# slinderman/theano_pyglm

Measured on AMD Instinct MI355X. Metric: population ll+grad evals/sec (N neurons x T bins), higher is better.
Workload: dtype f64

## Files before the change

theano_pyglm_amd/csrc/pglm_capi.hip:

```cpp
#include "pglm_kernels.hip.h"
#include "../../include/pyglm_hip.h"

#include <algorithm>
#include <cmath>
#include <cstdio>
#include <cstring>
#include <map>
#include <mutex>
#include <string>
#include <thread>
#include <type_traits>
#include <vector>

static thread_local std::string g_err;
static int fail(int code, const std::string& msg)
{
    g_err = msg;
    return code;
}
static thread_local std::vector<std::string>* g_dry = nullptr;
static thread_local std::vector<std::string>* g_rec = nullptr;
#define HIPCHK(expr)                                                                         \
    do {                                                                                     \
        hipError_t e_ = (expr);                                                              \
// ... 677 lines not shown
    sp.P = P; sp.Bt = h->sepBt; sp.Rt = h->sepRt; sp.npost = npost; sp.xs = xs;
    sp.Tstim = h->sepT; sp.nT = h->nT; sp.t_lo = t_lo; sp.t_hi = t_hi; sp.dt = h->dt; sp.dt_stim = h->sep_dt_stim;
    sp.X = X;
    const int nblk = (int)((t_hi - t_lo + PGL_SEP_TB - 1) / PGL_SEP_TB);
    hipLaunchKernelGGL(k_sep_conv_fwd, dim3(nblk, npost), dim3(256), (size_t)(2 * h->sepRt + PGL_SEP_TB) * 8,
                       h->stream, sp);
    HIPCHK(hipGetLastError());
    return PGL_OK;
}

static int sep_backward(pgl_handle h, const SepParams& sp, double* d_grad)
{
    if (g_dry) return PGL_OK;
    const int npost = sp.npost, Rt = h->sepRt;
    const int nblk = (int)((sp.t_hi - sp.t_lo + PGL_SEP_TB - 1) / PGL_SEP_TB);
    ENSURE(h->spart, (size_t)nblk * npost * Rt * 8);
    hipLaunchKernelGGL(k_sep_corr, dim3(nblk, npost), dim3(256), (size_t)(Rt + 2 * PGL_SEP_TB) * 8, h->stream, sp,
                       (double*)h->spart.p);
    HIPCHK(hipGetLastError());
    hipLaunchKernelGGL(k_sep_wt_grad, dim3(npost), dim3(64), 0, h->stream, sp, (const double*)h->spart.p, nblk,
                       d_grad);
    HIPCHK(hipGetLastError());
    const long long s_lo = std::max<long long>(0, sp.t_lo - Rt), nS = sp.t_hi - s_lo;
    ENSURE(h->Qb, (size_t)npost * nS * 8);
    ENSURE(h->Qf, (size_t)npost * h->sepT * 8);
    const int nblk_s = (int)((nS + PGL_SEP_TB - 1) / PGL_SEP_TB);
    hipLaunchKernelGGL(k_sep_conv_bwd, dim3(nblk_s, npost), dim3(256), (size_t)(2 * Rt + PGL_SEP_TB) * 8, h->stream,
                       sp, (double*)h->Qb.p, s_lo, nS);
    HIPCHK(hipGetLastError());
    hipLaunchKernelGGL(k_sep_interp_T, dim3((unsigned)((h->sepT + 255) / 256), npost), dim3(256), 0, h->stream, sp,
                       (const double*)h->Qb.p, s_lo, nS, (double*)h->Qf.p);
    HIPCHK(hipGetLastError());
    return launch_gemm_nt(h, (const double*)h->Qf.p, (int)h->sepT, (const double*)h->zfT.p, (int)h->sepT,
                          d_grad + 1 + h->sepBt, sp.P, npost, h->sepBx, (int)h->sepT);
}

static int launch_gemm_mfma(pgl_handle h, const double* A, long long sam, long long sak, const double* B,
                            long long sbn, long long sbk, double* C, long long scm, long long scn, int M, int N, int K)
{
    const int mb = (M + 15) / 16;
    if ((long long)mb * ((N + 63) / 64) >= 128)
        return launch_gemm_mfma_nt<4>(h, A, sam, sak, 0, B, sbn, sbk, 0, C, scm, scn, 0, M, N, K, 1);
    return launch_gemm_mfma_nt<1>(h, A, sam, sak, 0, B, sbn, sbk, 0, C, scm, scn, 0, M, N, K, 1);
}

static int launch_sepf_any(pgl_handle h, int which, const SepfParams& sp)
{
    if (h->sepJ == 5 && h->sepBTp == 3) launch_sepf<5, 3>(which, sp, h->stream);
    else launch_sepf<8, 4>(which, sp, h->stream);
    HIPCHK(hipGetLastError());
    return PGL_OK;
}

static int sepf_forward(pgl_handle h, const Plan& pl, const double* d_theta, SepfParams& sp, bool fused_fwd)
{
    if (g_dry) return PGL_OK;
    const int P = 1 + h->Dstim + h->Kimp, ldy = pl.nPT * 16;
    ENSURE(h->YfT, (size_t)h->sepT * ldy * 8);
    int rc = PGL_OK;
    const double* wx = d_theta + 1 + h->sepBt;
    if (gemm_aligned(h->zf.p, h->sepBx) && gemm_aligned(wx, P)) {
        rc = launch_gemm_kc<4, 1, 8>(h, (const double*)h->zf.p, (long long)h->sepBx, wx, (long long)P, (double*)h->YfT.p,
                                     (long long)ldy, 1LL, (int)h->sepT, pl.npost, h->sepBx);
    } else {
        rc = launch_gemm_mfma(h, wx, P, 1, (const double*)h->zfT.p, 1, h->sepT, (double*)h->YfT.p, 1, ldy, pl.npost,
                              (int)h->sepT, h->sepBx);
    }
    if (rc) return rc;
    sp.Ctab = (const double*)h->sepC.p; sp.YfT = (const double*)h->YfT.p; sp.theta = d_theta;
    sp.X = (double*)h->Xbuf.p; sp.Hb = nullptr; sp.wpart = nullptr; sp.QvT = nullptr; sp.grad = nullptr;
    sp.D = nullptr; sp.B0 = sp.B1 = 0; sp.SL = 0; sp.tilesPerChunk = 0;
    sp.P = P; sp.Bt = h->sepBt; sp.M = h->sepM; sp.q = h->sepq; sp.npost = pl.npost; sp.nPT = pl.nPT; sp.ldy = ldy;
    sp.tile0 = pl.tile0; sp.nTiles = pl.nTiles; sp.Tstim = h->sepT;
    const long long tb = (long long)pl.tile0 * 16, te = tb + (long long)pl.nTiles * 16;
    sp.F0 = tb / h->sepq; sp.F1 = (te - 1) / h->sepq;
    if (fused_fwd) return PGL_OK;
    return launch_sepf_any(h, 0, sp);
}

static int sepf_backward(pgl_handle h, SepfParams& sp, double* d_grad, bool fused_bwd = false, int* nwt = nullptr)
{
    if (g_dry) return PGL_OK;
    const long long nF = sp.F1 - sp.F0 + 1;
    ENSURE(h->QvT, (size_t)h->sepT * sp.ldy * 8);
    int rc = PGL_OK;
    if (fused_bwd) {
        const int nblk = (int)((h->sepT + 15) / 16);
        ENSURE(h->wpart, (size_t)nblk * 3 * sp.ldy * 8);
        sp.wpart = (double*)h->wpart.p; sp.QvT = (double*)h->QvT.p; sp.grad = d_grad;
        hipLaunchKernelGGL(k_sepf_finish_d, dim3((unsigned)nblk), dim3(1024), 0, h->stream, sp);
        HIPCHK(hipGetLastError());
        if (nwt) *nwt = nblk;
    } else {
        ENSURE(h->Hb, (size_t)nF * h->sepJ * sp.ldy * 8);
        ENSURE(h->wpart, (size_t)nF * h->sepBTp * sp.ldy * 8);
        sp.Hb = (double*)h->Hb.p; sp.wpart = (double*)h->wpart.p; sp.QvT = (double*)h->QvT.p; sp.grad = d_grad;
        rc = launch_sepf_any(h, 1, sp);
        if (!rc) rc = launch_sepf_any(h, 2, sp);
    }
    if (rc) return rc;
    if (gemm_aligned(h->zfT.p, h->sepT)) {
        return launch_gemm_kc<1, 0, 16>(h, (const double*)h->zfT.p, (long long)h->sepT, (const double*)h->QvT.p,
                                        (long long)sp.ldy, d_grad + 1 + h->sepBt, 1LL, (long long)sp.P, h->sepBx, sp.npost,
                                        (int)h->sepT);
    }
    return launch_gemm_mfma(h, (const double*)h->zf.p, 1, h->sepBx, (const double*)h->QvT.p, 1, sp.ldy,
                            d_grad + 1 + h->sepBt, 1, sp.P, h->sepBx, sp.npost, (int)h->sepT);
}

int pgl_sta(pgl_handle h, const double* stim, int64_t Tstim, int D, double dt_stim, int L,
            const int* neurons, int n_sel, double* A_out)
{
    if (!h || !stim) return fail(PGL_ERR_ARG, "null argument");
    if (!h->have_spikes) return fail(PGL_ERR_STATE, "pgl_set_spikes_* has not been called");
    if (Tstim <= 0 || D <= 0 || L <= 0 || !(dt_stim > 0)) return fail(PGL_ERR_ARG, "bad stimulus description");
    const int nSel = neurons ? n_sel : h->N;
    if (nSel <= 0 || nSel > 65535) return fail(PGL_ERR_ARG, "bad neuron selection");
    std::vector<int> eoff((size_t)2 * nSel);
    for (int i = 0; i < nSel; ++i) {
        const int n = neurons ? neurons[i] : i;
        if (n < 0 || n >= h->N) return fail(PGL_ERR_ARG, "neuron index out of range");
        eoff[2 * i] = h->h_ptr[n];
        eoff[2 * i + 1] = h->h_ptr[n + 1];
    }
    const long long LD = (long long)L * D;
    const long long xb = (LD + 255) / 256;
    if (xb > 0x7fffffffLL) return fail(PGL_ERR_UNSUPPORTED, "L*D too large");
    int echunks = (int)std::min<long long>(64, std::max<long long>(1, 4096 / (xb * nSel)));
    HIPCHK(hipSetDevice(h->device));
    DevBuf dstim, distim, deoff, dpart, dA;
    auto cleanup = [&]() { release(dstim); release(distim); release(deoff); release(dpart); release(dA); };
    auto keep = [&]() {
        release(h->staA);
        h->staA = dA;
        dA = DevBuf();
        h->sta_n = nSel; h->sta_L = L; h->sta_D = D;
    };
    const double ratio = dt_stim / h->dt;
    const long long q = llround(ratio);
    const bool frame_rate = q >= 1 && std::fabs(ratio - (double)q) <= 1e-9 * ratio && (Tstim % 2) == 0 && Tstim >= 2 &&
                            (long long)nSel * L * Tstim <= (1ll << 28) && h->opt_sepf != 7;
    int rc = ensure(dstim, (size_t)Tstim * D * 8);
    if (!rc && !frame_rate) rc = ensure(distim, (size_t)h->nT * D * 8);
    if (!rc) rc = ensure(deoff, eoff.size() * sizeof(int));
    if (!rc && !frame_rate) rc = ensure(dpart, (size_t)echunks * nSel * LD * 8);
    if (!rc) rc = ensure(dA, (size_t)nSel * LD * 8);
    if (rc) { cleanup(); return rc; }
    hipError_t e = hipMemcpyAsync(dstim.p, stim, (size_t)Tstim * D * 8, hipMemcpyHostToDevice, h->stream);
    if (e == hipSuccess)
        e = hipMemcpyAsync(deoff.p, eoff.data(), eoff.size() * sizeof(int), hipMemcpyHostToDevice, h->stream);
    if (frame_rate && e == hipSuccess) {
        DevBuf dW, dscale;
        std::vector<double> scale((size_t)nSel);
        for (int i = 0; i < nSel; ++i) {
            double cnt = 0.0;
            for (int j = eoff[2 * i]; j < eoff[2 * i + 1]; ++j) cnt += (double)h->h_ev[j].y;
            scale[i] = (h->dt / dt_stim) / cnt;
        }
        rc = ensure(dW, (size_t)nSel * L * Tstim * 8);
        if (!rc) rc = ensure(dscale, (size_t)nSel * 8);
// ... 280 lines not shown
                           (const uint8_t*)h->S.p, h->N, n_lo, p0.npost, (long long)h->t_lo, (long long)h->t_hi, rows, h->nlin,
                           h->dt, (double*)h->tmpA.p, (double*)h->tmpB.p, h->cur_pidx);
    HIPCHK(hipGetLastError());
    if (rr.row1 > h->t_hi) {
        hipLaunchKernelGGL(k_rows_zero, dim3(64), dim3(256), 0, h->stream, (double*)h->Xbuf.p, rr.xs, (long long)h->t_hi, rr.row1);
        HIPCHK(hipGetLastError());
    }
    hipLaunchKernelGGL(k_rows_reduce, dim3(p0.npost), dim3(64), 0, h->stream, (const double*)h->tmpA.p,
                       (const double*)h->tmpB.p, nblk, p0.npost, 1 + h->Dstim + h->Kimp, d_ll, d_out);
    HIPCHK(hipGetLastError());
    return PGL_OK;
}

static int backward_slices(pgl_handle h, const std::vector<Slice>& slices, const std::vector<Plan>& plans, int n_lo,
                           const double* d_theta, const double* d_Weff, double* d_ll, double* d_out)
{
    for (size_t i = 0; i < slices.size(); ++i) {
        int rc = launch_prep(h, plans[i], slices[i], n_lo, d_theta, d_Weff);
        if (rc) return rc;
        FusedParams fp;
        fill_params(h, plans[i], slices[i], n_lo, true, 2, fp);
        hipError_t e = launch_plan(plans[i], fp, h->stream);
        if (e != hipSuccess) return fail(PGL_ERR_HIP, std::string("backward launch: ") + hipGetErrorString(e));
        rc = launch_finalize_grad(h, plans[i], slices[i], n_lo, d_Weff, d_ll, d_out);
        if (rc) return rc;
    }
    return PGL_OK;
}

static int enqueue_ll_grad(pgl_handle h, int n_lo, int n_hi, const double* d_theta,
                           const double* d_Weff, double* d_ll, double* d_grad)
{
    KernelRecord record(h);
    std::vector<Slice> slices;
    std::vector<Plan> plans;
    bool sepf = false, sliced = false, wide = false;
    {
        int rc = select_plans(h, n_lo, n_hi, slices, plans, sepf, sliced, &wide);
        if (rc) return rc;
    }
    {
        int rc = ensure_partials(h, plans, d_grad != nullptr);
        if (rc) return rc;
    }

    const bool rec = h->opt_timing > 0 && (h->call_no++ % h->opt_timing) == 0;
    if (rec) {
        h->ev = h->evr[h->ev_launches % pgl_context::NEV];
        HIPCHK(hipEventRecord(h->ev[0], h->stream));
    }
    if (sepf) {
        const Plan& pl = plans[0];
        const bool direct = plan_reads_theta(pl);
        int rc = direct ? PGL_OK : launch_prep(h, pl, slices[0], n_lo, d_theta, d_Weff);
        if (rc) return rc;
        ENSURE(h->Xbuf, (size_t)pl.nTiles * pl.nPT * 256 * 8);
        rc = ensure_plan_images(h, pl);
        if (rc) return rc;
        if (rec) HIPCHK(hipEventRecord(h->ev[1], h->stream));
        SepfParams sp{};
        const bool fused_fwd = pl.version == 7 && fused7_built(pl.KT, pl.nw7, 2) && h->sepA_ok && h->opt_sepf != 3;
        const bool fused_bwd = fused_fwd && d_grad && fused7_built(pl.KT, pl.nw7, 3) && h->opt_sepf != 4;
        rc = sepf_forward(h, pl, d_theta, sp, fused_fwd);
        if (rc) return rc;
        if (fused_bwd && !g_dry) {
            const long long q = h->sepq, M = h->sepM;
            const long long tE = (long long)pl.tile0 + pl.nTiles - 1;
            sp.B0 = std::max<long long>(((long long)pl.tile0 * 16) / q - M, 0);
            sp.B1 = std::max<long long>((tE * 16) / q - M, 0);
            const long long span = ((M + 1) * q + 15) / 16 + 1;
            sp.SL = (int)(span / pl.tilesPerChunk) + 2;
            sp.tilesPerChunk = pl.tilesPerChunk;
            ENSURE(h->sepD, (size_t)(sp.B1 - sp.B0 + 1) * sp.SL * pl.nPT * 320 * 8);
            sp.D = (const double*)h->sepD.p;
        }
        FusedParams fp;
        fill_params(h, pl, slices[0], n_lo, d_grad != nullptr, 0, fp);
        if (direct) {
            fp.theta = d_theta;
            fp.Weff = d_Weff;
        }
        if (fused_fwd) {
            fp.sepA = (const double*)h->sepA.p; fp.sepZ = sp.YfT; fp.sepTheta = d_theta; fp.sepT = h->sepT;
            fp.sepLdy = sp.ldy; fp.sepQ = h->sepq; fp.sepM = h->sepM; fp.sepNH = h->sepNH; fp.sepG = h->sepGs;
            fp.sepBt = h->sepBt;
        }
        if (fused_bwd) {
            fp.sepAT = (const double*)h->sepAT.p; fp.sepD = (double*)h->sepD.p; fp.sepB0 = sp.B0; fp.sepSL = sp.SL;
        }
        hipError_t e = hipSuccess;
        if (pl.version == 5) {
            e = launch_fused5(pl, fp, h->stream, 1, 1);
            if (e == hipSuccess && d_grad) e = launch_fused5(pl, fp, h->stream, 2);
        } else {
            e = launch_fused7(pl, fp, h->stream, fused_bwd ? 3 : (fused_fwd ? 2 : 1));
        }
        if (e != hipSuccess) return fail(PGL_ERR_HIP, std::string("fused launch: ") + hipGetErrorString(e));
        if (d_grad) {
            int nwt = 0;
            rc = sepf_backward(h, sp, d_grad, fused_bwd, &nwt);
            if (rc) return rc;
            if (rec) HIPCHK(hipEventRecord(h->ev[2], h->stream));
            rc = launch_finalize_grad(h, pl, slices[0], n_lo, d_Weff, d_ll, d_grad, true, 0, -1, nullptr,
                                      fused_bwd ? (const double*)h->wpart.p : nullptr, nwt, sp.ldy);
            if (rc) return rc;
        } else {
            if (rec) HIPCHK(hipEventRecord(h->ev[2], h->stream));
            rc = launch_finalize_ll(h, pl, d_ll, d_grad);
            if (rc) return rc;
        }
    } else if (!sliced) {
        const Plan& pl = plans[0];
        const bool direct = plan_reads_theta(pl);
        int rc = direct ? PGL_OK : launch_prep(h, pl, slices[0], n_lo, d_theta, d_Weff);
        if (rc) return rc;
        if ((pl.version == 4 || pl.version == 5) && d_grad) {
            rc = ensure_tile_slab(h, pl);
            if (rc) return rc;
        }
        rc = ensure_plan_images(h, pl);
        if (rc) return rc;
        FusedParams fp;
        fill_params(h, pl, slices[0], n_lo, d_grad != nullptr, 0, fp);
        if (direct) {
            fp.theta = d_theta;
            fp.Weff = d_Weff;
        }
        if (rec) HIPCHK(hipEventRecord(h->ev[1], h->stream));
        hipError_t e = launch_plan(pl, fp, h->stream);
        if (e != hipSuccess) return fail(PGL_ERR_HIP, std::string("fused launch: ") + hipGetErrorString(e));
        if (rec) HIPCHK(hipEventRecord(h->ev[2], h->stream));
        rc = d_grad ? launch_finalize_grad(h, pl, slices[0], n_lo, d_Weff, d_ll, d_grad, true) : launch_finalize_ll(h, pl, d_ll, d_grad);
        if (rc) return rc;
    } else if (wide) {
        const Plan& p0 = plans[0];
        const size_t S = slices.size();
        ENSURE(h->Xbuf, (size_t)p0.nTiles * p0.nPT * 256 * 8);
        std::vector<int> slot(S);
        for (size_t i = 0; i < S; ++i) {
            int rc = ensure_feature_images(h, plans[i].ktl, plans[i].kth, p0.tile0, p0.nTiles, &slices[i], (int)i);
            if (rc) return rc;
            slot[i] = h->img_cur;
        }
        if (rec) HIPCHK(hipEventRecord(h->ev[1], h->stream));
        auto params = [&](const size_t i, FusedParams& fp) {
            h->img_cur = slot[i];
            fill_params(h, plans[i], slices[i], n_lo, d_grad != nullptr, 0, fp);
        };
        for (size_t i = 0; i < S; ++i) {
            int rc = launch_prep(h, plans[i], slices[i], n_lo, d_theta, d_Weff);
            if (rc) return rc;
// ... 1566 lines not shown
```

theano_pyglm_amd/csrc/pglm_reduce.hip.h:

```cpp
#pragma once
__global__ void k_prep_w(const double* __restrict__ theta, const double* __restrict__ Weff,
                         double* __restrict__ Wfrag, double* __restrict__ bias, int N, int B,
                         int Dstim, int Kimp, int Ktot, int KS, int n_lo, int npost, int nPT,
                         int pair, int Nall, int np0, int DsAll, int ds0, const int* __restrict__ pidx)
{
    const int P = 1 + DsAll + Nall * B;
    const long long total = (long long)nPT * KS * 64;
    for (long long i = blockIdx.x * (long long)blockDim.x + threadIdx.x; i < total;
         i += (long long)gridDim.x * blockDim.x) {
        const int lane = (int)(i & 63);
        const int ks = (int)((i >> 6) % KS);
        const int pt = (int)((i >> 6) / KS);
        const int k = 4 * ks + (lane >> 4);
        const int n = 16 * pt + (lane & 15);
        double v = 0.0;
        if (n < npost && k < Ktot) {
            if (k < Kimp) {
                const int npre = np0 + k / B;
                v = theta[(size_t)n * P + 1 + DsAll + np0 * B + k] * Weff[(size_t)npre * Nall + (pidx ? pidx[n] : n_lo + n)];
            } else {
                v = theta[(size_t)n * P + 1 + ds0 + (k - Kimp)];
            }
        }
        const long long o = pair ? (((long long)pt * (KS / 2) + (ks >> 1)) * 64 + lane) * 2 + (ks & 1) : i;
        Wfrag[o] = v;
    }
    for (int n = blockIdx.x * blockDim.x + threadIdx.x; n < nPT * 16; n += gridDim.x * blockDim.x)
        bias[n] = (n < npost) ? theta[(size_t)n * P] : 0.0;
}

__device__ __forceinline__ void pgl_reduce_ll(const double* __restrict__ llpart, const double* __restrict__ gbpart,
                                              double* __restrict__ ll_out, double* __restrict__ grad_out,
                                              const int n, const int P, const int nPT, const int nChunks,
                                              const int nsub, double (*red)[64])
{
    const int nthr = 256, t = (int)threadIdx.x, lane = t & 63, w = t >> 6, nw = 4;
    const int total = nChunks * nsub;
    const double* __restrict__ lp = llpart + (size_t)n * total;
    const double* __restrict__ gp = gbpart + (size_t)n * total;
    double sl[4] = {0.0, 0.0, 0.0, 0.0}, sg[4] = {0.0, 0.0, 0.0, 0.0};
    for (int i0 = t; i0 < total && t < nthr; i0 += 4 * nthr) {
#pragma unroll
        for (int j = 0; j < 4; ++j) {
            const int i = i0 + j * nthr;
            if (i < total) {
                sl[j] += lp[i];
                sg[j] += gp[i];
            }
        }
    }
    double a = (sl[0] + sl[1]) + (sl[2] + sl[3]), b = (sg[0] + sg[1]) + (sg[2] + sg[3]);
    for (int o = 32; o > 0; o >>= 1) {
        a += __shfl_xor(a, o, 64);
        b += __shfl_xor(b, o, 64);
    }
    if (lane == 0 && w < nw) {
        red[w][0] = a;
        red[w][1] = b;
    }
    __syncthreads();
    if (t == 0) {
        double x = 0.0, y = 0.0;
        for (int j = 0; j < nw; ++j) {
            x += red[j][0];
            y += red[j][1];
        }
        ll_out[n] = x;
        if (grad_out != nullptr) grad_out[(size_t)n * P] = y;
    }
}

__global__ __launch_bounds__(1024) void k_finalize(const double* __restrict__ Gpart, const double* __restrict__ llpart,
                           const double* __restrict__ gbpart, const double* __restrict__ Weff,
                           double* __restrict__ ll_out, double* __restrict__ grad_out, int N, int B,
                           int Dstim, int Kimp, int Ktot, int KT, int n_lo, int npost, int nPT,
                           int nChunks, int Nall, int np0, int DsAll, int ds0, int nsub, int kt0,
                           int nkt, const int* __restrict__ pidx, const double* __restrict__ wtpart = nullptr,
                           int nwt = 0, int ldy = 0, int Bt = 0)
{
    const int P = 1 + DsAll + Nall * B;
    const int nwf = (int)(blockDim.x >> 6);
    const long long nfrag = (long long)nPT * nkt * 256;
    const int gblocks = (int)((nfrag + 63) / 64);
    __shared__ double red[16][64];
    if ((int)blockIdx.x >= gblocks) {
        if (nsub <= 0) return;
        const int n = (int)blockIdx.x - gblocks;
        if (n >= npost) {
            const int bt = n - npost;
            if (wtpart == nullptr || bt >= Bt || grad_out == nullptr) return;
            const int lane = (int)(threadIdx.x & 63), w = (int)(threadIdx.x >> 6);
            double a[4] = {0.0, 0.0, 0.0, 0.0};
            if (lane < ldy) {
                int i = w, u = 0;
                for (; i < nwt; i += nwf, ++u) a[u & 3] += wtpart[((size_t)i * 3 + bt) * ldy + lane];
            }
            red[w][lane] = (a[0] + a[1]) + (a[2] + a[3]);
            __syncthreads();
            if (w == 0 && lane < npost) {
                double v = 0.0;
                for (int j = 0; j < nwf; ++j) v += red[j][lane];
                grad_out[(size_t)lane * P + 1 + bt] = v;
            }
            return;
        }
        pgl_reduce_ll(llpart, gbpart, ll_out, grad_out, n, P, nPT, nChunks, nsub, red);
        return;
    }
    if (grad_out == nullptr) return;
    const int lane = (int)(threadIdx.x & 63), w = (int)(threadIdx.x >> 6);
    const long long gid = blockIdx.x * 64LL + lane;
    const int r = (int)((gid >> 6) & 3);
    const int kt = kt0 + (int)((gid >> 8) % nkt);
    const int pt = (int)((gid >> 8) / nkt);
    const int k = 16 * kt + (lane >> 4) + 4 * r;
    const int n = 16 * pt + (lane & 15);
    const bool live = gid < nfrag && n < npost && k < Ktot;
    double s = 0.0;
    if (live) {
        const int per = (nChunks + nwf - 1) / nwf;
        const int c0 = w * per, c1 = (c0 + per < nChunks) ? c0 + per : nChunks;
        const double* gp = Gpart + (((size_t)pt * KT + kt) * 4 + r) * ((size_t)nChunks * 64) + lane;
        double a[8] = {0.0, 0.0, 0.0, 0.0, 0.0, 0.0, 0.0, 0.0};
        int c = c0;
        for (; c + 8 <= c1; c += 8) {
#pragma unroll
            for (int j = 0; j < 8; ++j) a[j] += gp[(size_t)(c + j) * 64];
        }
        for (int j = 0; c < c1; ++c, ++j) a[j] += gp[(size_t)c * 64];
        s = ((a[0] + a[1]) + (a[2] + a[3])) + ((a[4] + a[5]) + (a[6] + a[7]));
    }
    red[w][lane] = s;
    __syncthreads();
    if (w == 0 && live) {
        s = 0.0;
        for (int j = 0; j < nwf; ++j) s += red[j][lane];
        if (k < Kimp) {
            const int npre = np0 + k / B;
            grad_out[(size_t)n * P + 1 + DsAll + np0 * B + k] = s * Weff[(size_t)npre * Nall + (pidx ? pidx[n] : n_lo + n)];
        } else {
            grad_out[(size_t)n * P + 1 + ds0 + (k - Kimp)] = s;
        }
    }
}

__global__ __launch_bounds__(256) void k_finalize_ll(const double* __restrict__ llpart,
                                                     const double* __restrict__ gbpart,
                                                     double* __restrict__ ll_out,
                                                     double* __restrict__ grad_out, int P, int npost,
                                                     int nPT, int nChunks, int nsub)
{
    __shared__ double red[16][64];
    const int n = blockIdx.x;
    if (n >= npost) return;
    pgl_reduce_ll(llpart, gbpart, ll_out, grad_out, n, P, nPT, nChunks, nsub, red);
}

__global__ __launch_bounds__(256) void k_rows_epilogue(double* __restrict__ Xbuf, int xstride,
                                                       const double* __restrict__ bias,
                                                       const uint8_t* __restrict__ S, int Nall,
                                                       int n_lo, int npost, long long t_lo,
                                                       long long t_hi, int rows, int nlin, double dt,
                                                       double* __restrict__ llp,
                                                       double* __restrict__ gbp,
                                                       const int* __restrict__ pidx)
{
    const int n = blockIdx.y * 256 + threadIdx.x;
    if (n >= npost) return;
    const long long t0 = t_lo + (long long)blockIdx.x * rows;
    long long t1 = t0 + rows;
    if (t1 > t_hi) t1 = t_hi;
    const double b = bias[n];
    double ll = 0.0, gb = 0.0;
    for (long long t = t0; t < t1; ++t) {
        const double x = Xbuf[t * xstride + n] + b;
        const double s = (double)S[t * Nall + (pidx ? pidx[n] : n_lo + n)];
        double term, res;
        pgl_rate_terms(x, s, nlin, dt, term, res, PGL_C);
        ll += term;
        gb += res;
        Xbuf[t * xstride + n] = res;
    }
    llp[(size_t)blockIdx.x * npost + n] = ll;
    gbp[(size_t)blockIdx.x * npost + n] = gb;
}

__global__ void k_rows_zero(double* __restrict__ Xbuf, int xstride, long long r0, long long r1)
{
    const long long total = (r1 - r0) * xstride;
    for (long long i = blockIdx.x * (long long)blockDim.x + threadIdx.x; i < total;
         i += (long long)gridDim.x * blockDim.x)
        Xbuf[r0 * xstride + i] = 0.0;
}

__global__ __launch_bounds__(64) void k_rows_reduce(const double* __restrict__ llp,
                                                    const double* __restrict__ gbp, int nblk,
// ... 19 lines not shown
```

theano_pyglm_amd/csrc/pglm_stim.hip.h:

```cpp
#pragma once
__global__ void k_stim_project(const double* __restrict__ stim, long long Tstim, int D,
                               double dt_stim, double dt, const double* __restrict__ basis_x,
                               int Bx, double* __restrict__ zx, long long nT)
{
    const long long total = nT * Bx;
    for (long long i = blockIdx.x * (long long)blockDim.x + threadIdx.x; i < total;
         i += (long long)gridDim.x * blockDim.x) {
        const long long t = i / Bx;
        const int bx = (int)(i - t * Bx);
        const double x = dt * (double)t;
        long long i0 = (long long)floor(x / dt_stim);
        if (i0 > Tstim - 2) i0 = Tstim - 2;
        if (i0 < 0) i0 = 0;
        while (i0 + 1 < Tstim - 1 && dt_stim * (double)(i0 + 1) <= x) ++i0;
        while (i0 > 0 && dt_stim * (double)i0 > x) --i0;
        const double x0 = dt_stim * (double)i0, x1 = dt_stim * (double)(i0 + 1);
        const bool beyond = (Tstim < 2) || (x >= dt_stim * (double)(Tstim - 1));
        double acc = 0.0;
        const int d_lo = (basis_x == nullptr) ? bx : 0;
        const int d_hi = (basis_x == nullptr) ? bx + 1 : D;
        for (int d = d_lo; d < d_hi; ++d) {
            double v;
            if (beyond) {
                v = stim[(Tstim - 1) * D + d];
// ... 379 lines not shown
__global__ __launch_bounds__(1024) void k_sepf_finish(const SepfParams p, const int nA, const int nG)
{
    __shared__ double red[16][64];
    const int lane = threadIdx.x & 63, wave = threadIdx.x >> 6;
    const long long nF = p.F1 - p.F0 + 1;
    if ((int)blockIdx.x < nA) {
        const int g = blockIdx.x % nG;
        const long long f = (long long)(blockIdx.x / nG) * 16 + wave;
        const int n = g * 64 + lane;
        if (f >= p.Tstim || n >= p.ldy) return;
        auto gather = [&](const long long fv) -> double {
            double a = 0.0;
#pragma unroll
            for (int j = 0; j < J; ++j) {
                const long long F = fv + p.M - j;
                if (F >= p.M && F >= p.F0 && F <= p.F1) a += p.Hb[((size_t)(F - p.F0) * J + j) * p.ldy + n];
            }
            if (fv < J)
                for (long long F = p.F0; F < p.M && F <= p.F1; ++F) a += p.Hb[((size_t)(F - p.F0) * J + fv) * p.ldy + n];
            return a;
        };
        double acc = gather(f);
        if (f == p.Tstim - 1) {
            long long fmax = p.F1 + 1;
            if (fmax < J - 1) fmax = J - 1;
            for (long long fv = f + 1; fv <= fmax; ++fv) acc += gather(fv);
        }
        p.QvT[(size_t)f * p.ldy + n] = acc;
    } else {
        const int b = blockIdx.x - nA;
        const int g = b % nG, bt = b / nG;
        const int n = g * 64 + lane;
        const long long nW = (nF + 3) / 4;
        double a[8] = {0.0, 0.0, 0.0, 0.0, 0.0, 0.0, 0.0, 0.0};
        if (n < p.ldy) {
            long long F = wave;
            for (; F + 16 * 7 < nW; F += 16 * 8) {
#pragma unroll
                for (int u = 0; u < 8; ++u) a[u] += p.wpart[((size_t)(F + 16 * u) * BT + bt) * p.ldy + n];
            }
            for (int u = 0; F < nW; F += 16, ++u) a[u & 7] += p.wpart[((size_t)F * BT + bt) * p.ldy + n];
        }
        red[wave][lane] = ((a[0] + a[1]) + (a[2] + a[3])) + ((a[4] + a[5]) + (a[6] + a[7]));
        __syncthreads();
        if (wave == 0 && n < p.npost && bt < p.Bt) {
            double v = 0.0;
#pragma unroll
            for (int w = 0; w < 16; ++w) v += red[w][lane];
            p.grad[(size_t)n * p.P + 1 + bt] = v;
        }
    }
}

__global__ __launch_bounds__(1024) void k_sepf_finish_d(const SepfParams p)
{
    __shared__ double red[16][3][64];
    const int lane = threadIdx.x & 63, wave = threadIdx.x >> 6;
    const int n = lane, pt = lane >> 4, col = lane & 15;
    const long long f = (long long)blockIdx.x * 16 + wave;
    const bool vn = n < p.ldy && pt < p.nPT;
    const long long tileE = (long long)p.tile0 + p.nTiles - 1;
    double dt[3] = {0.0, 0.0, 0.0};
    auto gather = [&](const long long fv) {
#pragma unroll
        for (int j = 0; j < 6; ++j) {
            const long long b = fv - j;
            if (b < p.B0 || b > p.B1) continue;
            const long long tf = pgl_sepd_first_tile(b, p.M, p.q, p.tile0);
            long long tl = ((b + 1 + p.M) * (long long)p.q + 15) / 16 - 1;
            if (tl > tileE) tl = tileE;
            const int c0 = (int)((tf - p.tile0) / p.tilesPerChunk), c1 = (int)((tl - p.tile0) / p.tilesPerChunk);
            for (int sl = 0; sl <= c1 - c0; ++sl) {
                const double* dp = p.D + ((((size_t)(b - p.B0) * p.SL + sl) * p.nPT + pt) * 5) * 64 + col;
#pragma unroll
                for (int bt = 0; bt < 3; ++bt) {
                    const int c = 3 * j + bt;
                    const int o = (c < 16) ? (c >> 2) * 64 + (c & 3) * 16 : 4 * 64 + (c - 16) * 16;
                    dt[bt] += dp[o];
                }
            }
        }
    };
    if (vn && f < p.Tstim) {
        gather(f);
        if (f == p.Tstim - 1)
            for (long long fv = f + 1; fv <= p.B1 + 5; ++fv) gather(fv);
    }
    double gw[3] = {0.0, 0.0, 0.0};
    if (vn && f < p.Tstim) {
        const bool vr = n < p.npost;
        const double z = p.YfT[(size_t)f * p.ldy + n];
        double q = 0.0;
#pragma unroll
        for (int bt = 0; bt < 3; ++bt) {
            const double w = (vr && bt < p.Bt) ? p.theta[(size_t)n * p.P + 1 + bt] : 0.0;
            q = fma(dt[bt], w, q);
            gw[bt] = dt[bt] * z;
        }
        p.QvT[(size_t)f * p.ldy + n] = q;
    }
#pragma unroll
    for (int bt = 0; bt < 3; ++bt) red[wave][bt][lane] = gw[bt];
    __syncthreads();
    if (wave < 3 && vn) {
        double v = 0.0;
#pragma unroll
        for (int w = 0; w < 16; ++w) v += red[w][wave][lane];
        p.wpart[((size_t)blockIdx.x * 3 + wave) * p.ldy + n] = v;
    }
}

template <int NT>
__global__ __launch_bounds__(512) void k_gemm_mfma(const double* __restrict__ A, long long sam, long long sak,
                                                   const double* __restrict__ Bm, long long sbn, long long sbk,
                                                   double* __restrict__ C, long long scm, long long scn,
                                                   int M, int Nn, int Kd, long long sAb = 0, long long sBb = 0,
                                                   long long sCb = 0)
{
    A += (size_t)blockIdx.z * sAb;
    Bm += (size_t)blockIdx.z * sBb;
    C += (size_t)blockIdx.z * sCb;
    constexpr int NWG = 8, KC = 8;
    __shared__ double red[NWG - 1][NT][4][64];
    const int lane = threadIdx.x & 63;
    const int wave = __builtin_amdgcn_readfirstlane(threadIdx.x >> 6);
    const int i = lane & 15, kk = lane >> 4;
    const int m0 = blockIdx.x * 16, n0 = blockIdx.y * 16 * NT;
    const double* ap = A + (size_t)((m0 + i < M) ? m0 + i : M - 1) * sam;
    const double* bp[NT];
#pragma unroll
    for (int t = 0; t < NT; ++t) bp[t] = Bm + (size_t)((n0 + 16 * t + i < Nn) ? n0 + 16 * t + i : Nn - 1) * sbn;
    d4_t acc[NT];
#pragma unroll
    for (int t = 0; t < NT; ++t) acc[t] = (d4_t){0.0, 0.0, 0.0, 0.0};
    const int nU = (Kd + 4 * KC - 1) / (4 * KC);
    double a[KC], b[NT][KC];
    auto fetch = [&](const int u) {
#pragma unroll
        for (int v = 0; v < KC; ++v) {
            const int k = 4 * KC * u + KC * kk + v;
            const bool ok = k < Kd;
            const size_t kc = ok ? k : 0;
            const double av = ap[kc * sak];
            a[v] = ok ? av : 0.0;
#pragma unroll
            for (int t = 0; t < NT; ++t) {
                const double bv = bp[t][kc * sbk];
                b[t][v] = ok ? bv : 0.0;
            }
        }
    };
    if (wave < nU) fetch(wave);
    for (int u = wave; u < nU; u += NWG) {
        double ca[KC], cb[NT][KC];
#pragma unroll
        for (int v = 0; v < KC; ++v) {
            ca[v] = a[v];
#pragma unroll
            for (int t = 0; t < NT; ++t) cb[t][v] = b[t][v];
        }
        if (u + NWG < nU) fetch(u + NWG);
#pragma unroll
        for (int v = 0; v < KC; ++v)
#pragma unroll
            for (int t = 0; t < NT; ++t) acc[t] = __builtin_amdgcn_mfma_f64_16x16x4f64(ca[v], cb[t][v], acc[t], 0, 0, 0);
    }
    if (wave > 0) {
#pragma unroll
        for (int t = 0; t < NT; ++t)
#pragma unroll
            for (int r = 0; r < 4; ++r) red[wave - 1][t][r][lane] = acc[t][r];
    }
    __syncthreads();
    if (wave == 0) {
#pragma unroll
        for (int t = 0; t < NT; ++t)
#pragma unroll
            for (int r = 0; r < 4; ++r) {
                double v = acc[t][r];
#pragma unroll
                for (int w = 0; w < NWG - 1; ++w) v += red[w][t][r][lane];
                const int m = m0 + kk + 4 * r, n = n0 + 16 * t + i;
                if (m < M && n < Nn) C[(size_t)m * scm + (size_t)n * scn] = v;
            }
    }
}

template <int NT, int BK, int NB>
__global__ __launch_bounds__(512) void k_gemm_kc(const double* __restrict__ A, long long lda,
                                                 const double* __restrict__ Bm, long long ldb,
                                                 double* __restrict__ C, long long scm, long long scn,
                                                 int M, int Nn, int Kd)
{
    constexpr int NWG = 8;
    __shared__ double red[NWG - 1][NT][4][64];
    const int lane = threadIdx.x & 63;
    const int wave = __builtin_amdgcn_readfirstlane(threadIdx.x >> 6);
    const int i = lane & 15, kk = lane >> 4;
    const int m0 = blockIdx.x * 16, n0 = blockIdx.y * 16 * NT;
    const double* ap = A + (size_t)((m0 + i < M) ? m0 + i : M - 1) * lda;
    const double* bp[NT];
#pragma unroll
    for (int t = 0; t < NT; ++t) {
        const int n = (n0 + 16 * t + i < Nn) ? n0 + 16 * t + i : Nn - 1;
        bp[t] = BK ? Bm + (size_t)n * ldb : Bm + n;
    }
    d4_t acc[NT];
#pragma unroll
    for (int t = 0; t < NT; ++t) acc[t] = (d4_t){0.0, 0.0, 0.0, 0.0};
    const int nC = (Kd + 7) / 8;
    const int cpw = (nC + NWG - 1) / NWG;
    const int c_beg = wave * cpw, c_end = (c_beg + cpw < nC) ? c_beg + cpw : nC;
    for (int cb = c_beg; cb < c_end; cb += NB) {
        pgl_d2 a2[NB], b2[NB][NT];
#pragma unroll
        for (int c = 0; c < NB; ++c) {
            const int k = 8 * (cb + c) + 2 * kk;
            const bool ok = (cb + c < c_end) && k < Kd;
            const size_t kc = ok ? k : 0;
            const pgl_d2 av = *reinterpret_cast<const pgl_d2*>(ap + kc);
            a2[c].x = ok ? av.x : 0.0;
            a2[c].y = ok ? av.y : 0.0;
#pragma unroll
            for (int t = 0; t < NT; ++t) {
                pgl_d2 bv;
                if (BK) {
                    bv = *reinterpret_cast<const pgl_d2*>(bp[t] + kc);
                } else {
                    bv.x = bp[t][kc * ldb];
                    bv.y = bp[t][(kc + 1) * ldb];
                }
                b2[c][t].x = ok ? bv.x : 0.0;
                b2[c][t].y = ok ? bv.y : 0.0;
            }
        }
#pragma unroll
        for (int c = 0; c < NB; ++c)
#pragma unroll
            for (int t = 0; t < NT; ++t) {
                acc[t] = __builtin_amdgcn_mfma_f64_16x16x4f64(a2[c].x, b2[c][t].x, acc[t], 0, 0, 0);
                acc[t] = __builtin_amdgcn_mfma_f64_16x16x4f64(a2[c].y, b2[c][t].y, acc[t], 0, 0, 0);
            }
    }
    if (wave > 0) {
#pragma unroll
        for (int t = 0; t < NT; ++t)
#pragma unroll
            for (int r = 0; r < 4; ++r) red[wave - 1][t][r][lane] = acc[t][r];
    }
    __syncthreads();
    if (wave == 0) {
#pragma unroll
        for (int t = 0; t < NT; ++t)
#pragma unroll
            for (int r = 0; r < 4; ++r) {
                double v = acc[t][r];
#pragma unroll
                for (int w = 0; w < NWG - 1; ++w) v += red[w][t][r][lane];
                const int m = m0 + kk + 4 * r, n = n0 + 16 * t + i;
                if (m < M && n < Nn) C[(size_t)m * scm + (size_t)n * scn] = v;
            }
    }
}

__global__ __launch_bounds__(256) void k_sta(const int2* __restrict__ spk, const int* __restrict__ eoff,
                                             const double* __restrict__ istim, int D, int L,
                                             double* __restrict__ part)
{
    __shared__ int2 ev[256];
    const int i = blockIdx.y, c = blockIdx.z, nSel = gridDim.y, echunks = gridDim.z;
    const long long LD = (long long)L * D;
    const long long o = (long long)blockIdx.x * 256 + threadIdx.x;
    const int l = (int)(o / D);
    const int d = (int)(o - (long long)l * D);
    const int e0 = eoff[2 * i], e1 = eoff[2 * i + 1];
    const int per = (e1 - e0 + echunks - 1) / echunks;
    const int a = e0 + c * per;
    const int b = min(e1, a + per);
    double acc = 0.0;
    for (int base = a; base < b; base += 256) {
        const int e = base + (int)threadIdx.x;
        ev[threadIdx.x] = (e < b) ? spk[e] : make_int2(0, 0);
        __syncthreads();
        const int m = min(256, b - base);
        if (o < LD) {
            for (int j = 0; j < m; ++j) {
                const int2 q = ev[j];
                const long long tt = (long long)q.x - l;
                if (tt >= 0) acc = fma((double)q.y, istim[tt * D + d], acc);
            }
        }
        __syncthreads();
    }
    if (o < LD) part[((size_t)c * nSel + i) * LD + o] = acc;
}

__global__ __launch_bounds__(256) void k_sta_finish(const double* __restrict__ part,
                                                    const int2* __restrict__ spk,
                                                    const int* __restrict__ eoff, long long LD,
                                                    int echunks, double scale, double* __restrict__ A)
{
    __shared__ double red[256];
    const int i = blockIdx.y, nSel = gridDim.y;
    double cnt = 0.0;
    for (int e = eoff[2 * i] + (int)threadIdx.x; e < eoff[2 * i + 1]; e += 256) cnt += (double)spk[e].y;
    red[threadIdx.x] = cnt;
    __syncthreads();
    for (int s = 128; s > 0; s >>= 1) {
        if ((int)threadIdx.x < s) red[threadIdx.x] += red[threadIdx.x + s];
        __syncthreads();
    }
    cnt = red[0];
    const long long o = (long long)blockIdx.x * 256 + threadIdx.x;
    if (o >= LD) return;
    double acc = 0.0;
// ... 123 lines not shown
```

Measured before the change: 315.8.

## Fold weight prep into forward GEMM and merge sepf tail kernels

Runs the prep-weights work as extra blocks of the stimulus-projection GEMM launch, so the two independent jobs share one kernel. The finish-d reduction and the finalize reduction are likewise combined into one launch, and the backward GEMM and the temporal-weight gradient reduction into another. The aim is to cut kernel launch count and the serialization gaps between small kernels in the sepf path. In exchange, the tail path is limited to at most 8 finalize waves, and the merged kernels use shared memory sized for the larger role, which may reduce occupancy.

```diff
diff --git a/theano_pyglm_amd/csrc/pglm_capi.hip b/theano_pyglm_amd/csrc/pglm_capi.hip
--- a/theano_pyglm_amd/csrc/pglm_capi.hip
+++ b/theano_pyglm_amd/csrc/pglm_capi.hip
@@ -753,14 +753,23 @@
     return PGL_OK;
 }
 
-static int sepf_forward(pgl_handle h, const Plan& pl, const double* d_theta, SepfParams& sp, bool fused_fwd)
+static int sepf_forward(pgl_handle h, const Plan& pl, const double* d_theta, SepfParams& sp, bool fused_fwd,
+                        const PrepParams* prep = nullptr)
 {
     if (g_dry) return PGL_OK;
     const int P = 1 + h->Dstim + h->Kimp, ldy = pl.nPT * 16;
     ENSURE(h->YfT, (size_t)h->sepT * ldy * 8);
     int rc = PGL_OK;
     const double* wx = d_theta + 1 + h->sepBt;
-    if (gemm_aligned(h->zf.p, h->sepBx) && gemm_aligned(wx, P)) {
+    if (prep) {
+        const GemmKcParams g = {(const double*)h->zf.p, (long long)h->sepBx, wx, (long long)P, (double*)h->YfT.p,
+                                (long long)ldy, 1LL, (int)h->sepT, pl.npost, h->sepBx};
+        const int gx = (int)((h->sepT + 15) / 16), gy = (pl.npost + 63) / 64;
+        const long long total = (long long)pl.nPT * pl.KS * 64;
+        const int nprep = (int)std::min<long long>((total + 511) / 512, 512);
+        hipLaunchKernelGGL(k_sepf_head, dim3((unsigned)(gx * gy + nprep)), dim3(512), 0, h->stream, g, gx, gy, *prep, nprep);
+        HIPCHK(hipGetLastError());
+    } else if (gemm_aligned(h->zf.p, h->sepBx) && gemm_aligned(wx, P)) {
         rc = launch_gemm_kc<4, 1, 8>(h, (const double*)h->zf.p, (long long)h->sepBx, wx, (long long)P, (double*)h->YfT.p,
                                      (long long)ldy, 1LL, (int)h->sepT, pl.npost, h->sepBx);
     } else {
@@ -807,6 +816,44 @@
     }
     return launch_gemm_mfma(h, (const double*)h->zf.p, 1, h->sepBx, (const double*)h->QvT.p, 1, sp.ldy,
                             d_grad + 1 + h->sepBt, 1, sp.P, h->sepBx, sp.npost, (int)h->sepT);
+}
+
+static bool sepf_head_folds(pgl_handle h, const double* d_theta)
+{
+    return gemm_aligned(h->zf.p, h->sepBx) && gemm_aligned(d_theta + 1 + h->sepBt, 1 + h->Dstim + h->Kimp);
+}
+
+static int finalize_waves(pgl_handle h, const Plan& pl)
+{
+    return std::max(4, h->opt_finw > 0 ? h->opt_finw : std::max(4, std::min(8, pl.nChunks / 32)));
+}
+
+static bool sepf_tail_folds(pgl_handle h, const Plan& pl)
+{
+    return gemm_aligned(h->zfT.p, h->sepT) && finalize_waves(h, pl) <= 8;
+}
+
+static int sepf_tail(pgl_handle h, const Plan& pl, const Slice& sl, int n_lo, SepfParams& sp, const double* d_Weff,
+                     double* d_ll, double* d_grad)
+{
+    if (g_dry) return PGL_OK;
+    const int nfd = (int)((h->sepT + 15) / 16), nwf = finalize_waves(h, pl);
+    ENSURE(h->QvT, (size_t)h->sepT * sp.ldy * 8);
+    ENSURE(h->wpart, (size_t)nfd * 3 * sp.ldy * 8);
+    sp.wpart = (double*)h->wpart.p; sp.QvT = (double*)h->QvT.p; sp.grad = d_grad;
+    const FinalizeParams fin = {(const double*)h->Gpart.p, (const double*)h->llpart.p, (const double*)h->gbpart.p, d_Weff, d_ll,
+                                d_grad, sl.Ns, h->B, sl.Ds, sl.Ns * h->B, sl.Ns * h->B + sl.Ds, pl.KT, n_lo, pl.npost, pl.nPT,
+                                pl.nChunks, h->N, sl.np0, h->Dstim, sl.ds0, pl.KSPLIT, 0, pl.KT, h->cur_pidx, nullptr, 0, 0, 0};
+    const int fblocks = pl.nPT * pl.KT * 4 + pl.npost;
+    hipLaunchKernelGGL(k_sepf_tail_reduce, dim3((unsigned)(nfd + fblocks)), dim3(1024), 0, h->stream, sp, nfd, fin, nwf);
+    HIPCHK(hipGetLastError());
+    const GemmKcParams g = {(const double*)h->zfT.p, (long long)h->sepT, (const double*)h->QvT.p, (long long)sp.ldy,
+                            d_grad + 1 + h->sepBt, 1LL, (long long)sp.P, h->sepBx, sp.npost, (int)h->sepT};
+    const int gx = (h->sepBx + 15) / 16, gy = (sp.npost + 15) / 16;
+    hipLaunchKernelGGL(k_sepf_tail_gemm, dim3((unsigned)(gx * gy + h->sepBt)), dim3(512), 0, h->stream, g, gx, gy,
+                       (const double*)h->wpart.p, d_grad, nfd, sp.ldy, pl.npost, sp.P, h->sepBt, nwf);
+    HIPCHK(hipGetLastError());
+    return PGL_OK;
 }
 
 int pgl_sta(pgl_handle h, const double* stim, int64_t Tstim, int D, double dt_stim, int L,
@@ -1193,8 +1240,17 @@
     if (sepf) {
         const Plan& pl = plans[0];
         const bool direct = plan_reads_theta(pl);
-        int rc = direct ? PGL_OK : launch_prep(h, pl, slices[0], n_lo, d_theta, d_Weff);
+        const bool head_fold = !direct && !g_dry && sepf_head_folds(h, d_theta);
+        int rc = (direct || head_fold) ? PGL_OK : launch_prep(h, pl, slices[0], n_lo, d_theta, d_Weff);
         if (rc) return rc;
+        PrepParams prep{};
+        if (head_fold) {
+            const Slice& sl = slices[0];
+            ENSURE(h->Wfrag, (size_t)pl.nPT * pl.KS * 64 * 8);
+            ENSURE(h->bias, (size_t)pl.nPT * 16 * 8);
+            prep = PrepParams{d_theta, d_Weff, (double*)h->Wfrag.p, (double*)h->bias.p, sl.Ns, h->B, sl.Ds, sl.Ns * h->B,
+                              sl.Ns * h->B + sl.Ds, pl.KS, n_lo, pl.npost, pl.nPT, h->N, sl.np0, h->Dstim, sl.ds0, h->cur_pidx};
+        }
         ENSURE(h->Xbuf, (size_t)pl.nTiles * pl.nPT * 256 * 8);
         rc = ensure_plan_images(h, pl);
         if (rc) return rc;
@@ -1202,7 +1258,7 @@
         SepfParams sp{};
         const bool fused_fwd = pl.version == 7 && fused7_built(pl.KT, pl.nw7, 2) && h->sepA_ok && h->opt_sepf != 3;
         const bool fused_bwd = fused_fwd && d_grad && fused7_built(pl.KT, pl.nw7, 3) && h->opt_sepf != 4;
-        rc = sepf_forward(h, pl, d_theta, sp, fused_fwd);
+        rc = sepf_forward(h, pl, d_theta, sp, fused_fwd, head_fold ? &prep : nullptr);
         if (rc) return rc;
         if (fused_bwd && !g_dry) {
             const long long q = h->sepq, M = h->sepM;
@@ -1237,7 +1293,11 @@
             e = launch_fused7(pl, fp, h->stream, fused_bwd ? 3 : (fused_fwd ? 2 : 1));
         }
         if (e != hipSuccess) return fail(PGL_ERR_HIP, std::string("fused launch: ") + hipGetErrorString(e));
-        if (d_grad) {
+        if (d_grad && fused_bwd && sepf_tail_folds(h, pl)) {
+            if (rec) HIPCHK(hipEventRecord(h->ev[2], h->stream));
+            rc = sepf_tail(h, pl, slices[0], n_lo, sp, d_Weff, d_ll, d_grad);
+            if (rc) return rc;
+        } else if (d_grad) {
             int nwt = 0;
             rc = sepf_backward(h, sp, d_grad, fused_bwd, &nwt);
             if (rc) return rc;
diff --git a/theano_pyglm_amd/csrc/pglm_reduce.hip.h b/theano_pyglm_amd/csrc/pglm_reduce.hip.h
--- a/theano_pyglm_amd/csrc/pglm_reduce.hip.h
+++ b/theano_pyglm_amd/csrc/pglm_reduce.hip.h
@@ -1,13 +1,14 @@
 #pragma once
-__global__ void k_prep_w(const double* __restrict__ theta, const double* __restrict__ Weff,
+__device__ __forceinline__ void pgl_prep_w_block(const double* __restrict__ theta, const double* __restrict__ Weff,
                          double* __restrict__ Wfrag, double* __restrict__ bias, int N, int B,
                          int Dstim, int Kimp, int Ktot, int KS, int n_lo, int npost, int nPT,
-                         int pair, int Nall, int np0, int DsAll, int ds0, const int* __restrict__ pidx)
+                         int pair, int Nall, int np0, int DsAll, int ds0, const int* __restrict__ pidx,
+                         const int bid, const int nblk)
 {
     const int P = 1 + DsAll + Nall * B;
     const long long total = (long long)nPT * KS * 64;
-    for (long long i = blockIdx.x * (long long)blockDim.x + threadIdx.x; i < total;
-         i += (long long)gridDim.x * blockDim.x) {
+    for (long long i = bid * (long long)blockDim.x + threadIdx.x; i < total;
+         i += (long long)nblk * blockDim.x) {
         const int lane = (int)(i & 63);
         const int ks = (int)((i >> 6) % KS);
         const int pt = (int)((i >> 6) / KS);
@@ -25,8 +26,17 @@
         const long long o = pair ? (((long long)pt * (KS / 2) + (ks >> 1)) * 64 + lane) * 2 + (ks & 1) : i;
         Wfrag[o] = v;
     }
-    for (int n = blockIdx.x * blockDim.x + threadIdx.x; n < nPT * 16; n += gridDim.x * blockDim.x)
+    for (int n = bid * blockDim.x + threadIdx.x; n < nPT * 16; n += nblk * blockDim.x)
         bias[n] = (n < npost) ? theta[(size_t)n * P] : 0.0;
+}
+
+__global__ void k_prep_w(const double* __restrict__ theta, const double* __restrict__ Weff,
+                         double* __restrict__ Wfrag, double* __restrict__ bias, int N, int B,
+                         int Dstim, int Kimp, int Ktot, int KS, int n_lo, int npost, int nPT,
+                         int pair, int Nall, int np0, int DsAll, int ds0, const int* __restrict__ pidx)
+{
+    pgl_prep_w_block(theta, Weff, Wfrag, bias, N, B, Dstim, Kimp, Ktot, KS, n_lo, npost, nPT, pair, Nall, np0, DsAll, ds0, pidx,
+                     (int)blockIdx.x, (int)gridDim.x);
 }
 
 __device__ __forceinline__ void pgl_reduce_ll(const double* __restrict__ llpart, const double* __restrict__ gbpart,
@@ -70,46 +80,60 @@
     }
 }
 
-__global__ __launch_bounds__(1024) void k_finalize(const double* __restrict__ Gpart, const double* __restrict__ llpart,
-                           const double* __restrict__ gbpart, const double* __restrict__ Weff,
-                           double* __restrict__ ll_out, double* __restrict__ grad_out, int N, int B,
-                           int Dstim, int Kimp, int Ktot, int KT, int n_lo, int npost, int nPT,
-                           int nChunks, int Nall, int np0, int DsAll, int ds0, int nsub, int kt0,
-                           int nkt, const int* __restrict__ pidx, const double* __restrict__ wtpart = nullptr,
-                           int nwt = 0, int ldy = 0, int Bt = 0)
-{
+struct FinalizeParams {
+    const double* Gpart; const double* llpart; const double* gbpart; const double* Weff;
+    double* ll_out; double* grad_out;
+    int N, B, Dstim, Kimp, Ktot, KT, n_lo, npost, nPT, nChunks, Nall, np0, DsAll, ds0, nsub, kt0, nkt;
+    const int* pidx;
+    const double* wtpart;
+    int nwt, ldy, Bt;
+};
+
+__device__ __forceinline__ void pgl_reduce_wt(const double* __restrict__ wtpart, double* __restrict__ grad_out, const int bt,
+                                              const int nwt, const int ldy, const int npost, const int P, const int nwf,
+                                              double (*red)[64])
+{
+    const int lane = (int)(threadIdx.x & 63), w = (int)(threadIdx.x >> 6);
+    double a[4] = {0.0, 0.0, 0.0, 0.0};
+    if (lane < ldy && w < nwf) {
+        int i = w, u = 0;
+        for (; i < nwt; i += nwf, ++u) a[u & 3] += wtpart[((size_t)i * 3 + bt) * ldy + lane];
+    }
+    if (w < 16) red[w][lane] = (a[0] + a[1]) + (a[2] + a[3]);
+    __syncthreads();
+    if (w == 0 && lane < npost) {
+        double v = 0.0;
+        for (int j = 0; j < nwf; ++j) v += red[j][lane];
+        grad_out[(size_t)lane * P + 1 + bt] = v;
+    }
+}
+
+__device__ __forceinline__ void pgl_finalize_block(const FinalizeParams& q, const int bid, const int nwf, double (*red)[64])
+{
+    const double* __restrict__ Gpart = q.Gpart;
+    const double* __restrict__ Weff = q.Weff;
+    double* __restrict__ grad_out = q.grad_out;
+    const int B = q.B, Kimp = q.Kimp, Ktot = q.Ktot, KT = q.KT, n_lo = q.n_lo, npost = q.npost, nPT = q.nPT, nChunks = q.nChunks,
+              Nall = q.Nall, np0 = q.np0, DsAll = q.DsAll, ds0 = q.ds0, nsub = q.nsub, kt0 = q.kt0, nkt = q.nkt;
+    const int* __restrict__ pidx = q.pidx;
     const int P = 1 + DsAll + Nall * B;
-    const int nwf = (int)(blockDim.x >> 6);
     const long long nfrag = (long long)nPT * nkt * 256;
     const int gblocks = (int)((nfrag + 63) / 64);
-    __shared__ double red[16][64];
-    if ((int)blockIdx.x >= gblocks) {
+    if (bid >= gblocks) {
         if (nsub <= 0) return;
-        const int n = (int)blockIdx.x - gblocks;
+        const int n = bid - gblocks;
         if (n >= npost) {
             const int bt = n - npost;
-            if (wtpart == nullptr || bt >= Bt || grad_out == nullptr) return;
-            const int lane = (int)(threadIdx.x & 63), w = (int)(threadIdx.x >> 6);
-            double a[4] = {0.0, 0.0, 0.0, 0.0};
-            if (lane < ldy) {
-                int i = w, u = 0;
-                for (; i < nwt; i += nwf, ++u) a[u & 3] += wtpart[((size_t)i * 3 + bt) * ldy + lane];
-            }
-            red[w][lane] = (a[0] + a[1]) + (a[2] + a[3]);
-            __syncthreads();
-            if (w == 0 && lane < npost) {
-                double v = 0.0;
-                for (int j = 0; j < nwf; ++j) v += red[j][lane];
-                grad_out[(size_t)lane * P + 1 + bt] = v;
-            }
+            if (q.wtpart == nullptr || bt >= q.Bt || grad_out == nullptr) return;
+            pgl_reduce_wt(q.wtpart, grad_out, bt, q.nwt, q.ldy, npost, P, nwf, red);
             return;
         }
-        pgl_reduce_ll(llpart, gbpart, ll_out, grad_out, n, P, nPT, nChunks, nsub, red);
+        pgl_reduce_ll(q.llpart, q.gbpart, q.ll_out, grad_out, n, P, nPT, nChunks, nsub, red);
         return;
     }
     if (grad_out == nullptr) return;
     const int lane = (int)(threadIdx.x & 63), w = (int)(threadIdx.x >> 6);
-    const long long gid = blockIdx.x * 64LL + lane;
+    const long long gid = bid * 64LL + lane;
     const int r = (int)((gid >> 6) & 3);
     const int kt = kt0 + (int)((gid >> 8) % nkt);
     const int pt = (int)((gid >> 8) / nkt);
@@ -130,7 +154,7 @@
         for (int j = 0; c < c1; ++c, ++j) a[j] += gp[(size_t)c * 64];
         s = ((a[0] + a[1]) + (a[2] + a[3])) + ((a[4] + a[5]) + (a[6] + a[7]));
     }
-    red[w][lane] = s;
+    if (w < 16) red[w][lane] = s;
     __syncthreads();
     if (w == 0 && live) {
         s = 0.0;
@@ -142,6 +166,20 @@
             grad_out[(size_t)n * P + 1 + ds0 + (k - Kimp)] = s;
         }
     }
+}
+
+__global__ __launch_bounds__(1024) void k_finalize(const double* __restrict__ Gpart, const double* __restrict__ llpart,
+                           const double* __restrict__ gbpart, const double* __restrict__ Weff,
+                           double* __restrict__ ll_out, double* __restrict__ grad_out, int N, int B,
+                           int Dstim, int Kimp, int Ktot, int KT, int n_lo, int npost, int nPT,
+                           int nChunks, int Nall, int np0, int DsAll, int ds0, int nsub, int kt0,
+                           int nkt, const int* __restrict__ pidx, const double* __restrict__ wtpart = nullptr,
+                           int nwt = 0, int ldy = 0, int Bt = 0)
+{
+    __shared__ double red[16][64];
+    const FinalizeParams q = {Gpart, llpart, gbpart, Weff, ll_out, grad_out, N, B, Dstim, Kimp, Ktot, KT, n_lo, npost, nPT,
+                              nChunks, Nall, np0, DsAll, ds0, nsub, kt0, nkt, pidx, wtpart, nwt, ldy, Bt};
+    pgl_finalize_block(q, (int)blockIdx.x, (int)(blockDim.x >> 6), red);
 }
 
 __global__ __launch_bounds__(256) void k_finalize_ll(const double* __restrict__ llpart,
diff --git a/theano_pyglm_amd/csrc/pglm_stim.hip.h b/theano_pyglm_amd/csrc/pglm_stim.hip.h
--- a/theano_pyglm_amd/csrc/pglm_stim.hip.h
+++ b/theano_pyglm_amd/csrc/pglm_stim.hip.h
@@ -455,12 +455,11 @@
     }
 }
 
-__global__ __launch_bounds__(1024) void k_sepf_finish_d(const SepfParams p)
-{
-    __shared__ double red[16][3][64];
+__device__ __forceinline__ void pgl_sepf_finish_d_block(const SepfParams& p, const int bid, double (*red)[3][64])
+{
     const int lane = threadIdx.x & 63, wave = threadIdx.x >> 6;
     const int n = lane, pt = lane >> 4, col = lane & 15;
-    const long long f = (long long)blockIdx.x * 16 + wave;
+    const long long f = (long long)bid * 16 + wave;
     const bool vn = n < p.ldy && pt < p.nPT;
     const long long tileE = (long long)p.tile0 + p.nTiles - 1;
     double dt[3] = {0.0, 0.0, 0.0};
@@ -509,8 +508,22 @@
         double v = 0.0;
 #pragma unroll
         for (int w = 0; w < 16; ++w) v += red[w][wave][lane];
-        p.wpart[((size_t)blockIdx.x * 3 + wave) * p.ldy + n] = v;
-    }
+        p.wpart[((size_t)bid * 3 + wave) * p.ldy + n] = v;
+    }
+}
+
+__global__ __launch_bounds__(1024) void k_sepf_finish_d(const SepfParams p)
+{
+    __shared__ double red[16][3][64];
+    pgl_sepf_finish_d_block(p, (int)blockIdx.x, red);
+}
+
+__global__ __launch_bounds__(1024) void k_sepf_tail_reduce(const SepfParams p, const int nfd, const FinalizeParams fin,
+                                                           const int nwf)
+{
+    __shared__ double red[16 * 3 * 64];
+    if ((int)blockIdx.x < nfd) pgl_sepf_finish_d_block(p, (int)blockIdx.x, reinterpret_cast<double (*)[3][64]>(red));
+    else pgl_finalize_block(fin, (int)blockIdx.x - nfd, nwf, reinterpret_cast<double (*)[64]>(red));
 }
 
 template <int NT>
@@ -590,17 +603,16 @@
 }
 
 template <int NT, int BK, int NB>
-__global__ __launch_bounds__(512) void k_gemm_kc(const double* __restrict__ A, long long lda,
-                                                 const double* __restrict__ Bm, long long ldb,
-                                                 double* __restrict__ C, long long scm, long long scn,
-                                                 int M, int Nn, int Kd)
+__device__ __forceinline__ void pgl_gemm_kc_block(const double* __restrict__ A, long long lda,
+                                                  const double* __restrict__ Bm, long long ldb,
+                                                  double* __restrict__ C, long long scm, long long scn,
+                                                  int M, int Nn, int Kd, const int bx, const int by, double (*red)[NT][4][64])
 {
     constexpr int NWG = 8;
-    __shared__ double red[NWG - 1][NT][4][64];
     const int lane = threadIdx.x & 63;
     const int wave = __builtin_amdgcn_readfirstlane(threadIdx.x >> 6);
     const int i = lane & 15, kk = lane >> 4;
-    const int m0 = blockIdx.x * 16, n0 = blockIdx.y * 16 * NT;
+    const int m0 = bx * 16, n0 = by * 16 * NT;
     const double* ap = A + (size_t)((m0 + i < M) ? m0 + i : M - 1) * lda;
     const double* bp[NT];
 #pragma unroll
@@ -664,6 +676,57 @@
                 if (m < M && n < Nn) C[(size_t)m * scm + (size_t)n * scn] = v;
             }
     }
+}
+
+template <int NT, int BK, int NB>
+__global__ __launch_bounds__(512) void k_gemm_kc(const double* __restrict__ A, long long lda,
+                                                 const double* __restrict__ Bm, long long ldb,
+                                                 double* __restrict__ C, long long scm, long long scn,
+                                                 int M, int Nn, int Kd)
+{
+    __shared__ double red[7][NT][4][64];
+    pgl_gemm_kc_block<NT, BK, NB>(A, lda, Bm, ldb, C, scm, scn, M, Nn, Kd, (int)blockIdx.x, (int)blockIdx.y, red);
+}
+
+struct GemmKcParams {
+    const double* A; long long lda;
+    const double* B; long long ldb;
+    double* C; long long scm, scn;
+    int M, N, K;
+};
+
+struct PrepParams {
+    const double* theta; const double* Weff; double* Wfrag; double* bias;
+    int N, B, Dstim, Kimp, Ktot, KS, n_lo, npost, nPT, Nall, np0, DsAll, ds0;
+    const int* pidx;
+};
+__global__ __launch_bounds__(512) void k_sepf_head(const GemmKcParams g, const int gx, const int gy, const PrepParams w,
+                                                   const int nprep)
+{
+    __shared__ double red[7][4][4][64];
+    const int bid = (int)blockIdx.x;
+    if (bid < gx * gy) {
+        pgl_gemm_kc_block<4, 1, 8>(g.A, g.lda, g.B, g.ldb, g.C, g.scm, g.scn, g.M, g.N, g.K, bid % gx, bid / gx, red);
+        return;
+    }
+    pgl_prep_w_block(w.theta, w.Weff, w.Wfrag, w.bias, w.N, w.B, w.Dstim, w.Kimp, w.Ktot, w.KS, w.n_lo, w.npost, w.nPT, 1,
+                     w.Nall, w.np0, w.DsAll, w.ds0, w.pidx, bid - gx * gy, nprep);
+}
+
+__global__ __launch_bounds__(512) void k_sepf_tail_gemm(const GemmKcParams g, const int gx, const int gy,
+                                                        const double* __restrict__ wtpart, double* __restrict__ grad_out,
+                                                        const int nwt, const int ldy, const int npost, const int P,
+                                                        const int Bt, const int nwf)
+{
+    __shared__ double red[7 * 4 * 64];
+    const int bid = (int)blockIdx.x;
+    if (bid < gx * gy) {
+        pgl_gemm_kc_block<1, 0, 16>(g.A, g.lda, g.B, g.ldb, g.C, g.scm, g.scn, g.M, g.N, g.K, bid % gx, bid / gx,
+                                    reinterpret_cast<double (*)[1][4][64]>(red));
+        return;
+    }
+    if (bid - gx * gy < Bt)
+        pgl_reduce_wt(wtpart, grad_out, bid - gx * gy, nwt, ldy, npost, P, nwf, reinterpret_cast<double (*)[64]>(red));
 }
 
 __global__ __launch_bounds__(256) void k_sta(const int2* __restrict__ spk, const int* __restrict__ eoff,
```

New measurement: 316.0 (median of 2 runs). Within noise of the previous version (+0.0%).
